# xfause/OpenGL_Ray_Tracing

Hardware: AMD Instinct MI355X
Metric: Mrays/sec + ms/frame (1 spp, 1080p) at 1/2/4/8 MI355X; CPU-ref spp-matched PSNR (higher is better)
Workload: dtype f32; 1 GPU; c2: OpenglRayTracing bunny scene (5k tris), 1080p, 1 spp/frame, Lambert; resolution=1920x1080, spp_per_frame=1, integrator=lambert, max_bounce=2, triangles=5004, bvh_nodes=2826, bvh_builder=sah, env=peppermint, traversal_tree=runtime (checked against uploaded), frame_kernel=path regeneration, frames_in_flight=2, hw_queues=4, frames_per_launch=12, parallelism=screen-tile x1

## Files before the change

opengl_ray_tracing_amd/csrc/pt_kernels.h:

```cpp
#pragma once
#include <hip/hip_runtime.h>
#include <stdint.h>

namespace pt {

#ifndef PT_BLOCK
#define PT_BLOCK 256
#endif
constexpr int BLOCK = PT_BLOCK;
#ifndef PT_LDS_STACK
#define PT_LDS_STACK 32
#endif
#ifndef PT_MIN_WAVES_LAMBERT
#define PT_MIN_WAVES_LAMBERT 3
#endif
#ifndef PT_COST_EMA
#define PT_COST_EMA 2
#endif
#ifndef PT_WIDE_SCENE_MB
#define PT_WIDE_SCENE_MB 48
#endif
constexpr int WIDE_WAVES = 3;
#ifndef PT_WIDE_REGEN_WAVES
#define PT_WIDE_REGEN_WAVES 4
// ... 5 lines not shown
constexpr int wideRegenWaves(int integrator) { return integrator == 2 ? PT_WIDE_REGEN_WAVES : PT_WIDE_REGEN_WAVES_U; }
#ifndef PT_WIDE_REGEN_WAVES_SMALL
#define PT_WIDE_REGEN_WAVES_SMALL 3
#endif
#ifndef PT_MIN_WAVES
#define PT_MIN_WAVES 1
#endif
#ifndef PT_MIN_WAVES_MIS
#define PT_MIN_WAVES_MIS 3
#endif
constexpr int LDS_STACK = PT_LDS_STACK;
#ifndef PT_LDS_NODES
#define PT_LDS_NODES 128
#endif
constexpr int LDS_NODES = PT_LDS_NODES;
#ifndef PT_SPLIT_PCT
#define PT_SPLIT_PCT 25
#endif
#ifndef PT_SPLIT_AUTO
#define PT_SPLIT_AUTO 1
#endif
#ifndef PT_WAVE_TRACE
#define PT_WAVE_TRACE 0
#endif
#ifndef PT_PHASE_STATS
#define PT_PHASE_STATS 0
#endif
constexpr int PHASE_WORDS = 24;
constexpr int WAVE_TRACE_WORDS = PT_PHASE_STATS ? PHASE_WORDS : 6;
#ifndef PT_NUM_QUEUES
#define PT_NUM_QUEUES 32
#endif
constexpr int CTL_LINE_INTS = 64;
constexpr int NUM_QUEUES = PT_NUM_QUEUES;
static_assert((NUM_QUEUES & (NUM_QUEUES - 1)) == 0 && NUM_QUEUES <= 64, "NUM_QUEUES: power of two <= 64");
constexpr int RAY_SHARDS = 64;
constexpr int RAY_SHARD_STRIDE = CTL_LINE_INTS / 2;
constexpr int MAX_SLOTS = 16;
constexpr size_t CTL_QUEUES = 0;
constexpr size_t CTL_STATS = (size_t)MAX_SLOTS * 64 * 256;
constexpr size_t CTL_RAYS = CTL_STATS + 256;
constexpr size_t CTL_BYTES = CTL_RAYS + (size_t)RAY_SHARDS * 256;
#ifndef PT_FAST_TREE
#define PT_FAST_TREE 1
#endif
#ifndef PT_WIDE4
#define PT_WIDE4 2
#endif
#ifndef PT_FUSED_SLABS
#define PT_FUSED_SLABS 1
#endif
#ifndef PT_ACCEL_LEAF
#define PT_ACCEL_LEAF 4
#endif
#ifndef PT_PACKETS
#define PT_PACKETS 1
#endif
constexpr int PKT_DEPTH = 128;
constexpr int PAIR_F4 = 7;
constexpr int HIT_F4 = 4;
constexpr int MAT_F4 = 5;
constexpr int W4_F4 = 8;
constexpr int LEAF_CNT_BITS = 5;
constexpr int REF_NONE = (int)0x80000000;
constexpr int MAX_LEAF = 1 << LEAF_CNT_BITS;
constexpr int MAX_TRIS = (1 << (31 - LEAF_CNT_BITS)) - 1;
// ... 30 lines not shown
  const float2* trig;
  const uint2* light;
  int w, h, res;
  int nt;
};

constexpr int COL_F = 3;
struct FrameRef {
  float* col;
  uint32_t sampleIndex;
};

struct RenderParams {
  SceneView scene;
  Env env;
  int width, height;
  uint32_t frameCounter;
  uint32_t sampleIndex;
  int maxBounce;
  float eye[3];
  float cam[16];
  float4* accum;
  float* col;
  int nFrames;
  uint32_t sampleStride;
  size_t colStride;
  const int* binStart;
  const int* binTris;
  const float4* binGeo;
  const float4* binBox;
  int binTilesX, binTilesY;
  int2* primHit;
  unsigned long long* primMask;
  int zeroQueue;
  int* queue;
  int perQueue;
  int numItems;
  int shardSize;
  int shardTiles;
  int shardsX;
  int rank, world;
  int* ovf;
  int ovfDepth;
  int packets;
  unsigned long long* stats;
  unsigned long long* rayShards;
  const int* tileOrder;
  int orderCap;
  int* tileCost;
  int* tileCostMax;
  unsigned long long* waveTrace;
};

struct TraceParams {
  SceneView scene;
  const float* rays;
  int n;
  float* t;
  int* tri;
  int* ovf;
  int ovfDepth;
};

constexpr int BASIC_MAX_DEPTH = 31;
struct BasicParams {
  const double* shapes;
// ... 53 lines not shown
struct BuildNode {
  float4 lo;
  float4 hi;
  float4 clo;
  float4 chi;
};
struct AccelBuild {
  float4* bvh = nullptr;
  float4* pairs = nullptr;
  int* order = nullptr;
  BuildNode* nodes = nullptr;
  int rootRef = REF_NONE, nDev = 0, depth = 0, nNodes = 0;
};
hipError_t buildAccelDevice(const float4* geo, int nTri, int leafSize, float inflate, float inflateRelAbs,
                            AccelBuild& out, hipStream_t s);
void freeAccelBuild(AccelBuild& a);
hipError_t collapseWide4Device(const BuildNode* nodes, int nNodes, int leafSize, float inflate, float inflateRelAbs,
                               float4** out, int* rootRef, int* nDev, int* depth, hipStream_t s);

hipError_t launchHdrCache(const float* hdr, int w, int h, float4* cache, float* scratch, hipStream_t s);
hipError_t launchEnvCompact(const float4* hdr, const float2* cache, int w, int h, uint2* hdr8, uint32_t* cache4,
                            int* bad, hipStream_t s);
hipError_t launchEnvPack(float4* hdr, const float4* cache, float2* samp, int n, hipStream_t s);
hipError_t launchEnvTrig(float2* trig, int w, int h, hipStream_t s);
hipError_t launchEnvLight(const Env& e, uint2* light, hipStream_t s);
hipError_t launchRender(const RenderParams& p, int integrator, int grid, hipStream_t s, bool cull, bool count,
                        bool wide = false);
constexpr int REORDER_MAX = 4096;
hipError_t launchReorder(int* cost, int* costMax, int* splitLg, int* ema, int* order, int perQueue, int orderCap,
                         int numItems, int group, int numWaves, int splitPct, hipStream_t s);
hipError_t renderBlocksPerCU(int integrator, bool cull, bool count, bool wide, int* nb);
constexpr int PRIM_MISS = -1, PRIM_RETRACE = -2, PRIM_TILE = -3;
hipError_t launchPrimary(const RenderParams& p, hipStream_t s);
struct RegenShape {
  bool wide = false;
  bool fullTree = false;
  bool small = false;
  int block = BLOCK;
  int blocksPerCU = 0;
  size_t dynLds = 0;
};
hipError_t regenShape(int integrator, bool cull, bool wide, int f4nDev, bool smallScene, RegenShape* out);
hipError_t launchRegen(const RenderParams& p, int integrator, int grid, hipStream_t s, bool cull, const RegenShape& r);
int regenLdsStack();
int regenTop4(const RegenShape& r, int integrator);
hipError_t launchTrace(const TraceParams& p, int grid, hipStream_t s, bool cull);
struct GuideParams {
  SceneView scene;
  int width, height;
  float eye[3];
  float cam[16];
  float4* posT;
  float4* nrmTri;
  float4* albedo;
  int* ovf;
  int ovfDepth;
};
hipError_t launchGuides(const GuideParams& p, int grid, hipStream_t s, bool cull);
struct AtrousParams {
  int width, height;
  int stride;
  const float4* in;
  const float4* tmIn;
  const float4* posT;
  const float4* nrmTri;
  const float4* albedo;
  float4* out;
  float4* tmOut;
  float sigmaZ;
  float colDen, albDen;
  int colOn, albOn;
  int normalLog2;
  float limit;
};
constexpr int ATROUS_TILE = 16;
constexpr int ATROUS_LDS_STRIDE = 2;
// ... 70 lines not shown
```

opengl_ray_tracing_amd/csrc/pt_kernels.hip:

```cpp
#include <hip/hip_runtime.h>

#include <stdint.h>

#include "pt_device.h"
#include "pt_kernels.h"
#include "pt_scene.h"
#include "pt_trace.h"

namespace pt {



template <class T>
__device__ V3 pathLambert(T& tr, const Env& env, Hit hit, int maxBounce, uint32_t& seed, Counters& C, bool count) {
  V3 Lo = v3(0, 0, 0), history = v3(1, 1, 1);
  for (int bounce = 0; bounce < maxBounce; bounce++) {
    V3 wi = toNormalHemisphere(sampleHemisphereRand(seed), hit.N);
    Hit nh;
    bool isHit = tr.closest(hit.P, wi, nh);
    float pdf = 1.0f / (2.0f * PT_PI);
    float cosine_i = fmaxf(0.0f, dot(wi, hit.N));
    V3 f_r = hit.m.baseColor / PT_PI;
    if (!isHit) {
      V3 sky = sampleHdr(env, wi);
// ... 243 lines not shown
  __shared__ float4 s_tri[PT_PASS_BIN_CAP * 4];
  __shared__ float4 s_box[PT_PASS_BIN_CAP * 2];
  __shared__ int s_idx[PT_PASS_BIN_CAP];
  const int fr = (int)(blockIdx.x % (unsigned)p.nFrames);
  const int w = (int)(blockIdx.x / (unsigned)p.nFrames);
  const int lane = threadIdx.x;
  if (p.zeroQueue && blockIdx.x == 0)
    for (int q = lane; q < NUM_QUEUES; q += 64) p.queue[q * CTL_LINE_INTS] = 0;
  const int sub = p.shardSize >> 3;
  const int j = w / p.shardTiles, s = w - j * p.shardTiles;
  const int g = j * p.world + p.rank;
  const int gy = g / p.shardsX, gx = g - gy * p.shardsX;
  const int px = gx * p.shardSize + (s % sub) * 8 + (lane & 7);
  const int py = gy * p.shardSize + (s / sub) * 8 + (lane >> 3);
  const bool valid = px < p.width && py < p.height;
  const int tx = (gx * p.shardSize + (s % sub) * 8) >> 3, ty = (gy * p.shardSize + (s / sub) * 8) >> 3;
  int b0 = 0, b1 = 0;
  if (tx < p.binTilesX && ty < p.binTilesY) {
    b0 = p.binStart[ty * p.binTilesX + tx];
    b1 = p.binStart[ty * p.binTilesX + tx + 1];
  }
  const int n = b1 - b0;
  int2* out = p.primHit + ((size_t)fr * p.numItems + w) * 64;
  unsigned long long* mask = p.primMask + (size_t)fr * p.numItems + w;
  FrameRef fp;
  fp.col = p.col ? p.col + (size_t)fr * p.colStride * COL_F : nullptr;
  fp.sampleIndex = p.sampleIndex + (uint32_t)fr * p.sampleStride;
  if (n > PT_PASS_BIN_CAP) {
    const unsigned long long m = __ballot(valid);
    if (valid) out[__popcll(m & ((1ull << lane) - 1ull))] = make_int2(PRIM_TILE, 0);
    if (lane == 0) *mask = m;
    return;
  }
  for (int t = lane >> 2; t < n; t += 16) {
    s_tri[4 * t + (lane & 3)] = p.binGeo[4 * (size_t)(b0 + t) + (lane & 3)];
    if ((lane & 3) < 2) s_box[2 * t + (lane & 3)] = p.binBox[2 * (size_t)(b0 + t) + (lane & 3)];
    else if ((lane & 3) == 2) s_idx[t] = p.binTris[b0 + t];
  }
  __syncthreads();
  uint32_t seed;
  const V3 dir = cameraRay(p, fp.sampleIndex, valid ? px : 0, valid ? py : 0, seed);
  const V3 eye = v3(p.eye[0], p.eye[1], p.eye[2]);
  float tbest = PT_INF;
  int best = -1;
  bool tie = false;
  for (int k = 0; k < n; k++) {
    float tt;
    const bool h = valid && triTest(s_tri[4 * k], s_tri[4 * k + 1], s_tri[4 * k + 2], s_tri[4 * k + 3], eye, dir,
                                    PT_INF, tt);
    if (h && tt == tbest) tie = true;
    if (h && tt < tbest) {
      tbest = tt;
      best = k;
    }
  }
  uint32_t rays = 0;
  int res = PRIM_MISS;
  if (valid) {
    res = best >= 0 ? s_idx[best] : PRIM_MISS;
    if (tie || (res >= 0 && !refReachableBox(p.scene, s_box[2 * best], s_box[2 * best + 1], eye, dir, tbest))) {
      res = PRIM_RETRACE;
    } else {
      rays = 1;
      if (res == PRIM_MISS) {
        Counters C = {0, 0, 0, 0, 0};
        accumulate(p, fp, px, py, sampleHdr(p.env, dir), C, false);
      }
    }
  }
  const bool need = valid && res != PRIM_MISS;
  const unsigned long long m = __ballot(need);
  if (need) out[__popcll(m & ((1ull << lane) - 1ull))] = make_int2(res, __float_as_int(tbest));
  if (lane == 0) *mask = m;
  addRays(p.rayShards, rays);
}

hipError_t launchPrimary(const RenderParams& p, hipStream_t s) {
  if (!p.primHit || !p.primMask || !p.binStart || !p.binGeo || !p.binBox || p.numItems <= 0) return hipErrorInvalidValue;
  hipLaunchKernelGGL(primaryKernel, dim3((unsigned)p.numItems * (unsigned)p.nFrames), dim3(64), 0, s, p);
  return hipGetLastError();
}

template <int INTEG, bool CULL, bool COUNT>
__device__ __forceinline__ void finishPixel(const RenderParams& p, const FrameRef& f, int px, int py, int tri, float t,
                                            Stack& st, Counters& C, const float4* top) {
  Tracer<CULL, COUNT> tr{p.scene, st, C, top};
  uint32_t seed;
  const uint32_t sampleIndex = f.sampleIndex;
  const V3 dir = cameraRay(p, sampleIndex, px, py, seed);
  const V3 eye = v3(p.eye[0], p.eye[1], p.eye[2]);
  Hit first;
  finishHit(p.scene, tri, eye, dir, t, first);
  V3 Li;
  if (INTEG == 0) Li = pathLambert(tr, p.env, first, p.maxBounce, seed, C, COUNT);
  else if (INTEG == 1) Li = pathDisneyUniform(tr, p.env, first, p.maxBounce, seed, C, COUNT);
  else Li = pathMIS(tr, p.env, first, p.maxBounce, seed, px, py, sampleIndex, C, COUNT);
  const V3 Le0 = INTEG == 2 ? emissiveOf(p.scene, tri) : first.m.emissive;
  accumulate(p, f, px, py, Le0 + Li, C, COUNT);
}

struct BHit {
  double distance;
  V3 P, N, color;
  bool emissive;
  double specularRate, roughness, refractRate, refractAngle, refractRoughness;
};
struct BRng {
  uint32_t seed;
  const double* rep;
  long long pos, end;
  bool over;
};
// ... 733 lines not shown
```

opengl_ray_tracing_amd/csrc/pt_regen.hip:

```cpp
#include <hip/hip_runtime.h>
#include <stdint.h>

#include "pt_device.h"
#include "pt_kernels.h"
#include "pt_trace.h"

namespace pt {

#ifndef PT_REGEN_LDS_STACK
#define PT_REGEN_LDS_STACK 16
#endif
constexpr int REGEN_LDS_STACK = PT_REGEN_LDS_STACK;
#ifndef PT_REGEN_YIELD
#define PT_REGEN_YIELD 40
#endif
#ifndef PT_REGEN_MIN_WAVES_U
#define PT_REGEN_MIN_WAVES_U 4
#endif
#ifndef PT_REGEN_MIN_WAVES_MIS
#define PT_REGEN_MIN_WAVES_MIS 1
#endif

#ifndef PT_REGEN_TOP4
#define PT_REGEN_TOP4 128
#endif
#ifndef PT_REGEN_TOP4_3
#define PT_REGEN_TOP4_3 128
#endif
constexpr int regenTop4W(int waves) { return waves == 3 ? PT_REGEN_TOP4_3 : PT_REGEN_TOP4; }

#ifndef PT_TILE_PRIM
#define PT_TILE_PRIM 1
#endif

enum : int { K_NONE = 0, K_PRIMARY = 1, K_BOUNCE = 2, K_SHADOW = 3 };

struct PathState {
  int px, py;
  int fr;
  int kind;
  int bounce;
  uint32_t seed;
  V3 o, d;
  V3 Lo, hist;
  V3 Le0;
  int mat0;
  V3 f_r;
  float cosL;
  float pdfB;
  V3 Lb;
  V3 shC;
  bool haveB;
};

__device__ __forceinline__ uint32_t sampleOf(const RenderParams& p, const PathState& s) {
  return p.sampleIndex + (uint32_t)s.fr * p.sampleStride;
}

__device__ __forceinline__ void writeAccum(const RenderParams& p, const PathState& s, V3 color) {
  const int px = s.px, py = s.py;
  if (p.col) {
    stCol(p.col + ((size_t)s.fr * p.colStride + shareIndex(p, px, py)) * COL_F, color.x, color.y, color.z);
    return;
  }
  float4* a = p.accum + (size_t)py * p.width + px;
  float4 old = ldStream(a);
  float w = 1.0f / (float)(p.frameCounter + 1u);
// ... 135 lines not shown
      float mis_weight = misWeight(s.pdfB, pdf_light);
      V3 cc = ((s.hist * mis_weight) * c) * s.f_r;
      s.Lo = s.Lo + (cc * s.cosL) / s.pdfB;
    } else {
      const float pdf = 1.0f / (2.0f * PT_PI);
      V3 sky = sampleHdr(p.env, s.d);
      s.Lo = s.Lo + ((s.hist * sky) * s.f_r * s.cosL) / pdf;
    }
    color = camEmission<INTEG>(p, s) + s.Lo;
    return false;
  }
  Hit hit;
  finishHit(S, tri, s.o, s.d, t, hit);
  const V3 Le = hit.m.emissive;
  if (primary) {
    if (INTEG == 2) s.mat0 = hit.matId;
    else s.Le0 = Le;
  } else {
    const float pdf = INTEG == 2 ? s.pdfB : 1.0f / (2.0f * PT_PI);
    s.Lo = s.Lo + ((s.hist * Le) * s.f_r * s.cosL) / pdf;
    s.hist = s.hist * ((s.f_r * s.cosL) / pdf);
  }
  if (continueFromHit<INTEG>(p, s, hit, primary ? 0 : s.bounce + 1)) return true;
  color = camEmission<INTEG>(p, s) + s.Lo;
  return false;
}

template <int INTEG, bool CULL, int WAVES = 0, bool W4 = false, int BS = BLOCK, bool FULL = false>
__global__ __launch_bounds__(BS, WAVES > 0 ? WAVES : (INTEG == 2 ? PT_REGEN_MIN_WAVES_MIS : PT_REGEN_MIN_WAVES_U)) void regenKernel(
    RenderParams p) {
  static_assert(!FULL || W4, "the LDS tree is the 4-wide one");
  static_assert(!FULL || PT_REGEN_YIELD > 0, "the whole LDS tree is walked by walk4Run (loadNode4Lds) only");
  constexpr bool TILE_PRIM = PT_TILE_PRIM && INTEG != 2;
  __shared__ int s_stack[REGEN_LDS_STACK * BS];
  StackT<REGEN_LDS_STACK, BS> st;
  st.init(s_stack, p.ovf, p.ovfDepth);
  st.reset();
  __shared__ unsigned s_drained;
  if (threadIdx.x == 0) s_drained = 0;
#if PT_LDS_NODES > 0
  constexpr int TOP4 = regenTop4W(WAVES);
  constexpr int TOPF4 = FULL ? 1 : (W4 && TOP4 * W4_F4 > LDS_NODES * 4) ? TOP4 * W4_F4 : LDS_NODES * 4;
  __shared__ float4 s_nodes[TOPF4];
  extern __shared__ float4 s_tree[];
  if (FULL) {
    const float4* src = p.scene.fbvh4;
    const int n = p.scene.f4nTop * W4_LDS_F4;
    for (int i = threadIdx.x; i < n; i += BS) s_tree[i] = src[W4_F4 * (i / W4_LDS_F4) + i % W4_LDS_F4];
  } else {
    const bool w4 = W4 && p.scene.fast;
    const float4* src = w4 ? p.scene.fbvh4 : p.scene.bvh;
    const int n = w4 ? p.scene.f4nTop * W4_F4 : p.scene.nTop * 4;
    for (int i = threadIdx.x; i < n; i += BS) s_nodes[i] = src[i];
  }
  __syncthreads();
  const float4* top = FULL ? s_tree : s_nodes;
#else
  __syncthreads();
  const float4* top = nullptr;
#endif
  Counters C = {0, 0, 0, 0, 0};
  const int lane = threadIdx.x & 63;
  const int home = blockIdx.x & (NUM_QUEUES - 1);
  const int sub = p.shardSize >> 3;
  TileCursor cur;
  cur.drained = &s_drained;
// ... 25 lines not shown
  const long long phStart = clock64();
#define PH_ADD(k, x)                                                         \
  do {                                                                       \
    const unsigned long long v_ = (unsigned long long)(x);  \
    const unsigned long long m_ = __ballot(1);                               \
    if (__lane_id() == __ffsll((unsigned long long)m_) - 1) ph[k] += v_;     \
  } while (0)
#else
  unsigned long long* ph = nullptr;
#define PH_ADD(k, x) \
  do {               \
  } while (0)
#endif
  while (true) {
#if PT_PHASE_STATS
    const long long phA = clock64();
#endif
    if constexpr (TILE_PRIM) {
      while (true) {
        bool pend = false;
        int2 hP = make_int2(0, 0);
#if PT_PHASE_STATS
        const long long phH = clock64();
#endif
        while (true) {
          PH_ADD(11, 1);
          const unsigned long long idle = __ballot(!active);
          if (idle == 0) break;
          if (cursor >= nValid) {
#if PT_PHASE_STATS
            const long long phC = clock64();
            PH_ADD(17, 1);
#endif
            const int item = cur.next(p.queue, p.perQueue, p.numItems, home, tileFr, p.nFrames);
            if (item < 0) {
              drained = true;
              break;
            }
            tile = item;
#if PT_WAVE_TRACE
            wTiles++;
            wLastClaim = wall_clock64();
#endif
            if (p.primHit) {
              const unsigned long long m = primTileMask(p, tileFr, tile);
              const uint32_t lo = __builtin_amdgcn_readfirstlane((uint32_t)m);
              const uint32_t hi = __builtin_amdgcn_readfirstlane((uint32_t)(m >> 32));
              if ((lane < 32 ? lo >> lane : hi >> (lane - 32)) & 1u)
                s_slot[__builtin_amdgcn_mbcnt_hi(hi, __builtin_amdgcn_mbcnt_lo(lo, 0u))] = (unsigned char)lane;
              nValid = __popc(lo) + __popc(hi);
              if (lane < nValid) s_hit[lane] = primTileEntries(p, tileFr, tile)[lane];
            } else {
              const int px = tilePx(p, tile, sub) + (lane & 7), py = tilePy(p, tile, sub) + (lane >> 3);
              const bool in = px < p.width && py < p.height;
              const unsigned long long valid = __ballot(in);
              if (in) {
                const int k = rankBelow(valid);
                s_slot[k] = (unsigned char)lane;
                s_hit[k] = make_int2(PRIM_RETRACE, 0);
              }
              nValid = __popcll(valid);
            }
            __builtin_amdgcn_fence(__ATOMIC_RELEASE, "wavefront");
            __builtin_amdgcn_wave_barrier();
            __builtin_amdgcn_fence(__ATOMIC_ACQUIRE, "wavefront");
            cursor = 0;
#if PT_PHASE_STATS
            PH_ADD(18, clock64() - phC);
#endif
            continue;
          }
          const int r = cursor + rankBelow(idle);
          if (!active && r < nValid) {
            const int slot = s_slot[r];
            const int2 h = s_hit[r];
            s.px = tilePx(p, tile, sub) + (slot & 7);
            s.py = tilePy(p, tile, sub) + (slot >> 3);
            s.fr = tileFr;
            active = true;
            pend = true;
// ... 2 lines not shown
          cursor = min(nValid, cursor + __popcll(idle));
        }
#if PT_PHASE_STATS
        PH_ADD(16, clock64() - phH);
        const long long phS = clock64();
        if (__ballot(pend)) {
          PH_ADD(21, 1);
          PH_ADD(20, __popcll(__ballot(pend)));
        }
#endif
        bool ended = false;
        if (pend) {
          startPath(p, s);
          if (hP.x >= 0) {
            V3 color;
            if (!advance<INTEG>(p, s, hP.x, __int_as_float(hP.y), color)) {
              writeAccum(p, s, color);
              active = false;
              ended = true;
            }
          }
        }
#if PT_PHASE_STATS
        PH_ADD(19, clock64() - phS);
#endif
        if (drained || __ballot(ended) == 0) break;
      }
    } else {
      while (true) {
        PH_ADD(11, 1);
        const unsigned long long idle = __ballot(!active);
        if (idle == 0) break;
        if (cursor >= 64) {
          const int item = cur.next(p.queue, p.perQueue, p.numItems, home, tileFr, p.nFrames);
          if (item < 0) break;
          tile = item;
          cursor = 0;
          if (p.primHit) {
            const unsigned long long m = primTileMask(p, tileFr, tile);
            tmaskLo = __builtin_amdgcn_readfirstlane((uint32_t)m);
            tmaskHi = __builtin_amdgcn_readfirstlane((uint32_t)(m >> 32));
          }
#if PT_WAVE_TRACE
          wTiles++;
          wLastClaim = wall_clock64();
#endif
        }
        const int slot = cursor + rankBelow(idle);
        if (!active && slot < 64) {
          const int px = tilePx(p, tile, sub) + (slot & 7);
          const int py = tilePy(p, tile, sub) + (slot >> 3);
          int2 h = make_int2(0, 0);
          if (p.primHit)
            h = primOfSlot((unsigned long long)tmaskHi << 32 | tmaskLo, primTileEntries(p, tileFr, tile), slot);
          if (px < p.width && py < p.height && !(p.primHit && h.x == PRIM_MISS)) {
            s.px = px;
            s.py = py;
            s.fr = tileFr;
            startPath(p, s);
            active = true;
            if (p.primHit && h.x >= 0) {
              V3 color;
              if (!advance<INTEG>(p, s, h.x, __int_as_float(h.y), color)) {
                writeAccum(p, s, color);
                active = false;
              }
            }
          }
        }
        cursor = min(64, cursor + __popcll(idle));
      }
    }
#if PT_PHASE_STATS
    PH_ADD(0, clock64() - phA);
#endif
// ... 138 lines not shown
}

template <int I>
static hipError_t launchRegenI(const RenderParams& p, int grid, hipStream_t s, bool cull, const RegenShape& r) {
  if constexpr (I != 2 && PT_REGEN_YIELD > 0) {
    if (r.fullTree) {
      hipLaunchKernelGGL((regenKernel<I, true, wideRegenWaves(I), true, FULL_BS, true>), dim3(grid), dim3(FULL_BS),
                         r.dynLds, s, p);
      return hipGetLastError();
    }
  }
  if (r.fullTree) return hipErrorInvalidValue;
  if constexpr (I == 2 && PT_WIDE_REGEN_WAVES_SMALL != PT_WIDE_REGEN_WAVES)
    if (r.wide && r.small) {
      hipLaunchKernelGGL((regenKernel<I, true, PT_WIDE_REGEN_WAVES_SMALL, true>), dim3(grid), dim3(BLOCK), 0, s, p);
      return hipGetLastError();
    }
  if (r.wide)
    hipLaunchKernelGGL((regenKernel<I, true, wideRegenWaves(I), true>), dim3(grid), dim3(BLOCK), 0, s, p);
  else if (cull) hipLaunchKernelGGL((regenKernel<I, true>), dim3(grid), dim3(BLOCK), 0, s, p);
  else hipLaunchKernelGGL((regenKernel<I, false>), dim3(grid), dim3(BLOCK), 0, s, p);
  return hipGetLastError();
}

hipError_t launchRegen(const RenderParams& p, int integrator, int grid, hipStream_t s, bool cull, const RegenShape& r) {
  if (r.fullTree && p.scene.f4nTop * W4_LDS_F4 * sizeof(float4) > r.dynLds) return hipErrorInvalidValue;
  switch (integrator) {
    case 0: return launchRegenI<0>(p, grid, s, cull, r);
    case 1: return launchRegenI<1>(p, grid, s, cull, r);
    default: return launchRegenI<2>(p, grid, s, cull, r);
  }
}

int regenLdsStack() { return REGEN_LDS_STACK; }
int regenTop4(const RegenShape& r, int integrator) {
  return regenTop4W(r.small ? PT_WIDE_REGEN_WAVES_SMALL : wideRegenWaves(integrator));
}

}
```

opengl_ray_tracing_amd/csrc/pt_runtime.cpp:

```cpp
#include <hip/hip_runtime.h>

#include <algorithm>
#include <array>
#include <map>
#include <chrono>
#include <cmath>
#include <cstdio>
#include <cstdlib>
#include <cstring>
#include <string>
#include <vector>

#include "pt_abi.h"
#include "pt_accel.h"
#include "pt_fmath.h"
#include "pt_kernels.h"
#include "pt_rccl.h"
#include "pt_scene.h"

using namespace pt;

static constexpr int EV_RING = 64;
#ifndef PT_PIPE
#define PT_PIPE 8
// ... 60 lines not shown
  uint32_t* d_cache4 = nullptr;
  uint32_t* d_cacheRow = nullptr;
  unsigned short* d_cacheY = nullptr;
  float2* d_trig = nullptr;
  uint2* d_light = nullptr;
  int hdrW = 0, hdrH = 0;
  double* d_shapes = nullptr;
  int nShapes = 0;
  double* d_basicImg = nullptr;
  double* d_stream = nullptr;
  long long* d_offsets = nullptr;
  long long streamN = 0, nOffsets = 0;
  unsigned long long* d_overruns = nullptr;
  float4* d_accum = nullptr;
  unsigned char* d_ctl = nullptr;
  int* d_ovf = nullptr;
  int* d_cost = nullptr;
  int* d_order = nullptr;
  bool lastFast = false;
  bool lastRegen = false;
  int lastWaves = 0;
  int probeFrame = 0;
  PrimaryBins bins;
  bool binsValid = false;
  float binEye[3] = {}, binCam[16] = {};
  unsigned sceneVersion = 0, binVersion = 0;
  bool pipe = false;
  int pipeDepth = PT_PIPE;
  int pipeDepthBase = PT_PIPE;
  bool pipeDepthFixed = false;
  int batchCap = 1;
  int colCap[COLS] = {};
  int primCap[PIPE] = {};
  int regenWide = -1;
  bool solo = true;
  hipStream_t slotStream[PIPE] = {};
  hipEvent_t kernelDone[PIPE] = {};
  bool slotBusy[PIPE] = {};
  hipEvent_t mixDone[COLS] = {};
  hipStream_t lastMixStream = nullptr;
  hipEvent_t binsBuilt = nullptr;
  unsigned binGen = 0, binGenSeen[MAX_SLOTS] = {};
  float* d_col[COLS] = {};
  int2* d_prim[PIPE] = {};
  int lastSlot = -1;
  int lastCol = -1;
  bool mixPending = false;
  unsigned long long frameNo = 0;
  int probeN[4] = {0, 0, 0, 0};
  double probeMs[4] = {0.0, 0.0, 0.0, 0.0};
  long long probeLast[4] = {-1, -1, -1, -1};
  int probeGen = 0;
  int treeDecided = -1, splitDecided = -1;
  unsigned policyKey = 0, probedKey = ~0u;
  int orderCap = 0;
  bool orderValid[PIPE] = {};
  bool orderSplit[PIPE] = {};
  size_t ovfInts = 0;
  int shardSize = 32, shardsX = 0, shardsY = 0, numItems = 0, perQueue = 0;
  float* d_rays = nullptr;
  float* d_t = nullptr;
  int* d_tri = nullptr;
  size_t traceCap = 0;
  float* d_rgb = nullptr;
  float4* d_guide[3] = {};
  float4* d_guidePN[2][2] = {};
  int guideSet = 0;
  float guideEye[3] = {}, guideCam[16] = {};
  bool guidesValid = false;
  unsigned guideVersion = 0;
  int* d_guideOvf = nullptr;
  size_t guideOvfInts = 0;
  float4* d_dn[2] = {};
  float4* d_dnTm[2] = {};
  const float4* denoised = nullptr;
  float4* d_res[2] = {};
  int resCur = 0;
// ... 243 lines not shown
    ctx->peers.push_back(p);
  }
  if ((rc = createGroup(ctx)) != PT_OK) {
    g_create_err = ctx->err;
    pt_destroy(ctx);
    *out = nullptr;
    return rc;
  }
  return PT_OK;
}

void pt_destroy(pt_ctx* ctx) {
  if (!ctx) return;
  destroyGroup(ctx);
  (void)hipSetDevice(ctx->cfg.device_id);
  if (ctx->own) (void)hipStreamSynchronize(ctx->own);
  dfree(ctx->d_geo); dfree(ctx->d_hit); dfree(ctx->d_mats); dfree(ctx->d_bvh); dfree(ctx->d_pairs);
  dfree(ctx->d_fbvh); dfree(ctx->d_fbvh4); dfree(ctx->d_fpairs); dfree(ctx->d_fastTri);
  dfree(ctx->d_refParent); dfree(ctx->d_refBox); dfree(ctx->d_leafBox);
  dfree(ctx->d_hdr); dfree(ctx->d_cache); dfree(ctx->d_hdr8); dfree(ctx->d_cache4); dfree(ctx->d_shapes);
  dfree(ctx->d_cacheRow); dfree(ctx->d_cacheY); dfree(ctx->d_trig); dfree(ctx->d_light);
  dfree(ctx->d_basicImg); dfree(ctx->d_stream); dfree(ctx->d_offsets); dfree(ctx->d_overruns);
  dfree(ctx->d_accum); dfree(ctx->d_ctl); dfree(ctx->d_ovf); dfree(ctx->d_cost); dfree(ctx->d_order);
  dfree(ctx->d_rays); dfree(ctx->d_t); dfree(ctx->d_tri); dfree(ctx->d_rgb);
  dfree(ctx->d_guide[2]);
  for (auto& set : ctx->d_guidePN) for (auto& g : set) dfree(g);
  dfree(ctx->d_res[0]); dfree(ctx->d_res[1]);
  dfree(ctx->d_mom); dfree(ctx->d_lum); dfree(ctx->d_var0); dfree(ctx->d_lv[0]); dfree(ctx->d_lv[1]);
  dfree(ctx->d_guideOvf); dfree(ctx->d_dn[0]); dfree(ctx->d_dn[1]); dfree(ctx->d_dnTm[0]); dfree(ctx->d_dnTm[1]);
  freePrimaryBins(ctx->bins);
  for (int k = 0; k < PIPE; k++) {
    if (ctx->slotStream[k]) (void)hipStreamSynchronize(ctx->slotStream[k]);
    dfree(ctx->d_prim[k]);
    if (ctx->kernelDone[k]) (void)hipEventDestroy(ctx->kernelDone[k]);
    if (ctx->slotStream[k]) (void)hipStreamDestroy(ctx->slotStream[k]);
  }
  for (int k = 0; k < COLS; k++) {
    dfree(ctx->d_col[k]);
    if (ctx->mixDone[k]) (void)hipEventDestroy(ctx->mixDone[k]);
  }
  if (ctx->binsBuilt) (void)hipEventDestroy(ctx->binsBuilt);
  for (hipEvent_t e : ctx->ev)
    if (e) (void)hipEventDestroy(e);
  if (ctx->own) (void)hipStreamDestroy(ctx->own);
  delete ctx;
}

static inline void nrm3(const float* a, const float* b, const float* c, float N[3]) {
  float e1x = b[0] - a[0], e1y = b[1] - a[1], e1z = b[2] - a[2];
  float e2x = c[0] - a[0], e2y = c[1] - a[1], e2z = c[2] - a[2];
  float cx = e1y * e2z - e2y * e1z;
  float cy = e1z * e2x - e2z * e1x;
  float cz = e1x * e2y - e2x * e1y;
  float inv = 1.0f / std::sqrt((cx * cx + cy * cy) + cz * cz);
  N[0] = cx * inv; N[1] = cy * inv; N[2] = cz * inv;
}

struct WideTree {
  std::vector<float4> bvh;
  int rootRef = REF_NONE, nDev = 0, depth = 0;
};

static std::string encodeWideTree(const float* nodes, int nNodes, int nTri, float inflate, WideTree& out,
                                  float inflateAbs = 0.0f) {
  auto nodeN = [&](int k) { return (int)nodes[(size_t)k * 12 + 3]; };
  auto isInternal = [&](int k) { return k > 0 && k < nNodes && nodeN(k) <= 0; };
// ... 1141 lines not shown
        ctx->binGenSeen[slot] = ctx->binGen;
      }
    }
    if (piped && ctx->binGenSeen[slot] != ctx->binGen) {
      CK(hipStreamWaitEvent(S, ctx->binsBuilt, 0));
      ctx->binGenSeen[slot] = ctx->binGen;
    }
    p.binStart = ctx->bins.binStart;
    p.binTris = ctx->bins.binTris;
    p.binGeo = ctx->bins.binGeo;
    p.binBox = ctx->bins.binBox;
    p.binTilesX = ctx->bins.tilesX;
    p.binTilesY = ctx->bins.tilesY;
    if (pass) {
      const size_t primBytes = shareN * sizeof(int2) + (size_t)ctx->numItems * sizeof(unsigned long long);
      if (piped)
        for (int k = 0; k < D; k++)
          if (!ctx->d_prim[k]) {
            const int cap = std::max(nF, ctx->batchCap);
            CK(hipMalloc(&ctx->d_prim[k], (size_t)cap * primBytes));
            ctx->primCap[k] = cap;
          }
      if (ctx->primCap[slot] < nF) {
        if (ctx->d_prim[slot]) {
          CK(hipStreamSynchronize(S));
          dfree(ctx->d_prim[slot]);
        }
        const int cap = std::max(nF, piped ? ctx->batchCap : 1);
        CK(hipMalloc(&ctx->d_prim[slot], (size_t)cap * primBytes));
        ctx->primCap[slot] = cap;
      }
      p.primHit = ctx->d_prim[slot];
      p.primMask = reinterpret_cast<unsigned long long*>(ctx->d_prim[slot] + (size_t)ctx->primCap[slot] * shareN);
    }
  }
  const bool splitThis = nF == 1;
  p.tileOrder = ordered && ctx->orderValid[slot] && !(!splitThis && ctx->orderSplit[slot]) ? order : nullptr;
  p.orderCap = orderCap;
  p.tileCost = ordered ? cost : nullptr;
  p.tileCostMax = ordered ? cost + ctx->numItems : nullptr;
  if (piped && probing) {
    if (int e = waitOthers()) return e;
  }
  int erc = launchEvents(ctx, &evb, &eve);
  if (erc) return erc;
#if PT_WAVE_TRACE
  const size_t nTrace = (size_t)grid * (bs / 64) * WAVE_TRACE_WORDS;
  unsigned long long* dTrace = nullptr;
  {
    CK(hipMalloc(&dTrace, nTrace * sizeof(unsigned long long)));
    CK(hipMemsetAsync(dTrace, 0, nTrace * sizeof(unsigned long long), S));
  }
  p.waveTrace = dTrace;
#endif
  p.zeroQueue = p.primHit != nullptr;
  if (!p.primHit) CK(hipMemsetAsync(queue, 0, (size_t)NUM_QUEUES * CTL_LINE_INTS * sizeof(int), S));
  CK(hipEventRecord(evb, S));
  if (p.primHit) CK(launchPrimary(p, S));
  if (regen) CK(launchRegen(p, c.integrator, grid, S, cull, rs));
  else CK(launchRender(p, c.integrator, grid, S, cull, count, wide));
#if PT_WAVE_TRACE
  if (dTrace) {
    std::vector<unsigned long long> tr(nTrace);
    CK(hipMemcpyAsync(tr.data(), dTrace, nTrace * sizeof(unsigned long long), hipMemcpyDeviceToHost, S));
    CK(hipStreamSynchronize(S));
    (void)hipFree(dTrace);
    if (const char* fn = std::getenv("PT_WAVE_TRACE_FILE")) {
      if (FILE* f = std::fopen(fn, "ab")) {
        std::fwrite(tr.data(), sizeof(unsigned long long), nTrace, f);
        std::fclose(f);
      }
    }
  }
#endif
  if (ordered) {
    CK(launchReorder(cost, cost + ctx->numItems, cost + 2 * (size_t)ctx->numItems, cost + 3 * (size_t)ctx->numItems,
                     order, ctx->perQueue, orderCap, ctx->numItems, group, grid * (BLOCK / 64), splitThis ? splitPct : 0, S));
    ctx->orderValid[slot] = true;
    ctx->orderSplit[slot] = splitThis && splitPct > 0;
  }
  CK(hipEventRecord(eve, S));
  if (piped) {
    CK(hipEventRecord(ctx->kernelDone[slot], S));
    ctx->slotBusy[slot] = true;
    if (S != ctx->slotStream[slot])
      CK(hipStreamWaitEvent(ctx->slotStream[slot], ctx->kernelDone[slot], 0));
    if (S != ctx->stream) CK(hipStreamWaitEvent(ctx->stream, ctx->kernelDone[slot], 0));
    if (ctx->mixPending && ctx->lastMixStream != ctx->stream)
      CK(hipStreamWaitEvent(ctx->stream, ctx->mixDone[ctx->lastCol], 0));
    ctx->lastMixStream = ctx->stream;
    if (ctx->d_mom) {
// ... 1012 lines not shown
```

opengl_ray_tracing_amd/csrc/pt_trace.h:

```cpp
#pragma once
#include "pt_device.h"
#include "pt_kernels.h"

namespace pt {

struct Counters {
  uint32_t rays, nodes, tris, mats, texels;
};

#ifndef PT_LEAF_WAIT_MK
#define PT_LEAF_WAIT_MK 0
#endif

template <int DEPTH, int STRIDE>
struct StackT {
  static_assert((DEPTH & (DEPTH - 1)) == 0, "LDS stack depth must be a power of two");
  static constexpr int HALF = DEPTH / 2;
  int* lds;
  int* ovf;
  int ovfDepth;
  int sp;
  int base;
  __device__ __forceinline__ void init(int* ldsBase, int* ovfArea, int depth) {
    lds = ldsBase + threadIdx.x;
// ... 666 lines not shown
struct TileCursor {
  int qi = 0;
  unsigned* drained = nullptr;
  __device__ __forceinline__ int next(int* queue, int perQueue, int numItems, int home, int& frame, int nFrames = 1,
                                      const int* order = nullptr, int orderCap = 0) {
    while (qi < NUM_QUEUES) {
      const int q = (home + qi) & (NUM_QUEUES - 1);
      if (drained && qi > 0 &&
          ((__builtin_amdgcn_readfirstlane(*(volatile unsigned*)drained) >> q) & 1u)) {
        qi++;
        continue;
      }
      int it = 0;
      if ((threadIdx.x & 63) == 0) it = atomicAdd(queue + q * CTL_LINE_INTS, 1);
      it = __builtin_amdgcn_readfirstlane(it);
      const int k = nFrames == 1 ? it : it / nFrames;
      if (order) {
        if (it < order[NUM_QUEUES * orderCap + q] * nFrames) {
          frame = it - k * nFrames;
          return order[q * orderCap + k];
        }
      } else {
        const int t = q * perQueue + k;
        if (k < perQueue && t < numItems) {
          frame = it - k * nFrames;
          return t;
        }
      }
      if (drained && (threadIdx.x & 63) == 0) atomicOr(drained, 1u << q);
      qi++;
    }
    return -1;
  }
};

__device__ __forceinline__ size_t shareIndex(const RenderParams& p, int px, int py) {
  const int ss = p.shardSize;
  const int gx = px / ss, gy = py / ss;
  const int j = (gy * p.shardsX + gx) / p.world;
  return (size_t)j * ss * ss + (size_t)((py - gy * ss) * ss + (px - gx * ss));
}

__device__ __forceinline__ unsigned long long primTileMask(const RenderParams& p, int fr, int w) {
  return p.primMask[(size_t)fr * p.numItems + w];
}
__device__ __forceinline__ const int2* primTileEntries(const RenderParams& p, int fr, int w) {
  return p.primHit + ((size_t)fr * p.numItems + w) * 64;
}
__device__ __forceinline__ int2 primOfSlot(unsigned long long m, const int2* e, int slot) {
  if (!((m >> slot) & 1ull)) return make_int2(PRIM_MISS, 0);
  return e[__popcll(m & ((1ull << slot) - 1ull))];
}

__device__ __forceinline__ void addRays(unsigned long long* shards, uint32_t r) {
  for (int off = 32; off > 0; off >>= 1) r += __shfl_down(r, off, 64);
  if ((threadIdx.x & 63) == 0 && r)
    atomicAdd(shards + (blockIdx.x & (RAY_SHARDS - 1)) * RAY_SHARD_STRIDE, (unsigned long long)r);
}

struct Hit {
  V3 P, N, viewDir;
  Material m;
  int matId;
};
__device__ __forceinline__ V3 emissiveMat(const SceneView& S, int matId) {
  const float4* m = S.mats + MAT_F4 * (size_t)matId;
// ... 102 lines not shown
```

Baseline: 20200 Mrays/s.

## Compact non-empty tiles into per-queue live lists before regen kernel

Adds a liveListKernel that scans primary-hit masks per queue and writes a compacted list of (tile, frame, mask) entries for tiles that have at least one live pixel. The regen kernel's work hand-out then claims entries from this list via nextLive, which skips empty (all-miss) tiles and reads the mask through the scalar constant path instead of a separate load. It also skips the bin load and barrier in the primary kernel when a bin is empty. The cost is one extra small kernel launch per batch, extra device buffers, and host-side allocation logic.

```diff
diff --git a/opengl_ray_tracing_amd/csrc/pt_kernels.h b/opengl_ray_tracing_amd/csrc/pt_kernels.h
--- a/opengl_ray_tracing_amd/csrc/pt_kernels.h
+++ b/opengl_ray_tracing_amd/csrc/pt_kernels.h
@@ -61,6 +61,8 @@
 #define PT_NUM_QUEUES 32
 #endif
 constexpr int CTL_LINE_INTS = 64;
+constexpr int LIVE_HEAD = 16;
+__host__ __device__ constexpr int liveStride(int perQueue, int nFrames) { return LIVE_HEAD + ((perQueue * nFrames + 15) & ~15); }
 constexpr int NUM_QUEUES = PT_NUM_QUEUES;
 static_assert((NUM_QUEUES & (NUM_QUEUES - 1)) == 0 && NUM_QUEUES <= 64, "NUM_QUEUES: power of two <= 64");
 constexpr int RAY_SHARDS = 64;
@@ -157,6 +159,7 @@
   int binTilesX, binTilesY;
   int2* primHit;
   unsigned long long* primMask;
+  uint4* liveItems;
   int zeroQueue;
   int* queue;
   int perQueue;
@@ -276,6 +279,7 @@
 hipError_t renderBlocksPerCU(int integrator, bool cull, bool count, bool wide, int* nb);
 constexpr int PRIM_MISS = -1, PRIM_RETRACE = -2, PRIM_TILE = -3;
 hipError_t launchPrimary(const RenderParams& p, hipStream_t s);
+hipError_t launchLiveList(const RenderParams& p, hipStream_t s);
 struct RegenShape {
   bool wide = false;
   bool fullTree = false;
@@ -286,6 +290,7 @@
 };
 hipError_t regenShape(int integrator, bool cull, bool wide, int f4nDev, bool smallScene, RegenShape* out);
 hipError_t launchRegen(const RenderParams& p, int integrator, int grid, hipStream_t s, bool cull, const RegenShape& r);
+bool regenTakesLists(int integrator, const RegenShape& r);
 int regenLdsStack();
 int regenTop4(const RegenShape& r, int integrator);
 hipError_t launchTrace(const TraceParams& p, int grid, hipStream_t s, bool cull);
diff --git a/opengl_ray_tracing_amd/csrc/pt_kernels.hip b/opengl_ray_tracing_amd/csrc/pt_kernels.hip
--- a/opengl_ray_tracing_amd/csrc/pt_kernels.hip
+++ b/opengl_ray_tracing_amd/csrc/pt_kernels.hip
@@ -299,12 +299,14 @@
     if (lane == 0) *mask = m;
     return;
   }
-  for (int t = lane >> 2; t < n; t += 16) {
-    s_tri[4 * t + (lane & 3)] = p.binGeo[4 * (size_t)(b0 + t) + (lane & 3)];
-    if ((lane & 3) < 2) s_box[2 * t + (lane & 3)] = p.binBox[2 * (size_t)(b0 + t) + (lane & 3)];
-    else if ((lane & 3) == 2) s_idx[t] = p.binTris[b0 + t];
-  }
-  __syncthreads();
+  if (n > 0) {
+    for (int t = lane >> 2; t < n; t += 16) {
+      s_tri[4 * t + (lane & 3)] = p.binGeo[4 * (size_t)(b0 + t) + (lane & 3)];
+      if ((lane & 3) < 2) s_box[2 * t + (lane & 3)] = p.binBox[2 * (size_t)(b0 + t) + (lane & 3)];
+      else if ((lane & 3) == 2) s_idx[t] = p.binTris[b0 + t];
+    }
+    __syncthreads();
+  }
   uint32_t seed;
   const V3 dir = cameraRay(p, fp.sampleIndex, valid ? px : 0, valid ? py : 0, seed);
   const V3 eye = v3(p.eye[0], p.eye[1], p.eye[2]);
@@ -345,6 +347,51 @@
 hipError_t launchPrimary(const RenderParams& p, hipStream_t s) {
   if (!p.primHit || !p.primMask || !p.binStart || !p.binGeo || !p.binBox || p.numItems <= 0) return hipErrorInvalidValue;
   hipLaunchKernelGGL(primaryKernel, dim3((unsigned)p.numItems * (unsigned)p.nFrames), dim3(64), 0, s, p);
+  return hipGetLastError();
+}
+
+constexpr int LIVE_BS = 1024;
+__global__ __launch_bounds__(LIVE_BS) void liveListKernel(RenderParams p) {
+  __shared__ int s_wave[LIVE_BS / 64];
+  const int q = blockIdx.x, lane = threadIdx.x & 63, wv = threadIdx.x >> 6;
+  const int nF = p.nFrames, total = p.perQueue * nF;
+  uint4* seg = p.liveItems + (size_t)q * liveStride(p.perQueue, nF);
+  uint4* out = seg + LIVE_HEAD;
+  auto load = [&](int it, int& t, int& fr) -> unsigned long long {
+    const int k = it / nF;
+    fr = it - k * nF;
+    t = q * p.perQueue + k;
+    return it < total && t < p.numItems ? p.primMask[(size_t)fr * p.numItems + t] : 0ull;
+  };
+  int base = 0;
+  int t, fr;
+  unsigned long long m = load((int)threadIdx.x, t, fr);
+  for (int it0 = 0; it0 < total; it0 += LIVE_BS) {
+    int tn, frn;
+    const unsigned long long mn = load(it0 + LIVE_BS + (int)threadIdx.x, tn, frn);
+    const unsigned long long b = __ballot(m != 0);
+    if (lane == 0) s_wave[wv] = __popcll(b);
+    __syncthreads();
+    int before = 0, all = 0;
+    for (int w = 0; w < LIVE_BS / 64; w++) {
+      const int c = s_wave[w];
+      before += w < wv ? c : 0;
+      all += c;
+    }
+    if (m != 0)
+      out[base + before + __popcll(b & ((1ull << lane) - 1ull))] = make_uint4((uint32_t)t, (uint32_t)fr, (uint32_t)m, (uint32_t)(m >> 32));
+    base += all;
+    __syncthreads();
+    m = mn;
+    t = tn;
+    fr = frn;
+  }
+  if (threadIdx.x == 0) seg[0] = make_uint4((uint32_t)base, 0u, 0u, 0u);
+}
+
+hipError_t launchLiveList(const RenderParams& p, hipStream_t s) {
+  if (!p.primMask || !p.liveItems || p.numItems <= 0) return hipErrorInvalidValue;
+  hipLaunchKernelGGL(liveListKernel, dim3(NUM_QUEUES), dim3(LIVE_BS), 0, s, p);
   return hipGetLastError();
 }
 
diff --git a/opengl_ray_tracing_amd/csrc/pt_regen.hip b/opengl_ray_tracing_amd/csrc/pt_regen.hip
--- a/opengl_ray_tracing_amd/csrc/pt_regen.hip
+++ b/opengl_ray_tracing_amd/csrc/pt_regen.hip
@@ -33,6 +33,9 @@
 #define PT_TILE_PRIM 1
 #endif
 
+constexpr bool regenLists(int integ, int waves) {
+  return !(integ == 2 && waves == PT_WIDE_REGEN_WAVES && PT_WIDE_REGEN_WAVES_SMALL != PT_WIDE_REGEN_WAVES);
+}
 enum : int { K_NONE = 0, K_PRIMARY = 1, K_BOUNCE = 2, K_SHADOW = 3 };
 
 struct PathState {
@@ -234,6 +237,7 @@
   static_assert(!FULL || W4, "the LDS tree is the 4-wide one");
   static_assert(!FULL || PT_REGEN_YIELD > 0, "the whole LDS tree is walked by walk4Run (loadNode4Lds) only");
   constexpr bool TILE_PRIM = PT_TILE_PRIM && INTEG != 2;
+  constexpr bool LISTS = regenLists(INTEG, WAVES);
   __shared__ int s_stack[REGEN_LDS_STACK * BS];
   StackT<REGEN_LDS_STACK, BS> st;
   st.init(s_stack, p.ovf, p.ovfDepth);
@@ -325,20 +329,18 @@
             const long long phC = clock64();
             PH_ADD(17, 1);
 #endif
-            const int item = cur.next(p.queue, p.perQueue, p.numItems, home, tileFr, p.nFrames);
-            if (item < 0) {
+            uint32_t lo = 0, hi = 0;
+            static_assert(LISTS, "the tile hand-out's variants all take live lists");
+            if (!cur.nextLive(p.queue, p.primHit ? p.liveItems : nullptr, p.perQueue, p.numItems, p.nFrames, home, tile,
+                              tileFr, lo, hi)) {
               drained = true;
               break;
             }
-            tile = item;
 #if PT_WAVE_TRACE
             wTiles++;
             wLastClaim = wall_clock64();
 #endif
             if (p.primHit) {
-              const unsigned long long m = primTileMask(p, tileFr, tile);
-              const uint32_t lo = __builtin_amdgcn_readfirstlane((uint32_t)m);
-              const uint32_t hi = __builtin_amdgcn_readfirstlane((uint32_t)(m >> 32));
               if ((lane < 32 ? lo >> lane : hi >> (lane - 32)) & 1u)
                 s_slot[__builtin_amdgcn_mbcnt_hi(hi, __builtin_amdgcn_mbcnt_lo(lo, 0u))] = (unsigned char)lane;
               nValid = __popc(lo) + __popc(hi);
@@ -407,15 +409,21 @@
         const unsigned long long idle = __ballot(!active);
         if (idle == 0) break;
         if (cursor >= 64) {
-          const int item = cur.next(p.queue, p.perQueue, p.numItems, home, tileFr, p.nFrames);
-          if (item < 0) break;
-          tile = item;
+          if constexpr (LISTS) {
+            if (!cur.nextLive(p.queue, p.primHit ? p.liveItems : nullptr, p.perQueue, p.numItems, p.nFrames, home, tile,
+                              tileFr, tmaskLo, tmaskHi))
+              break;
+          } else {
+            const int item = cur.next(p.queue, p.perQueue, p.numItems, home, tileFr, p.nFrames);
+            if (item < 0) break;
+            tile = item;
+            if (p.primHit) {
+              const unsigned long long m = primTileMask(p, tileFr, tile);
+              tmaskLo = __builtin_amdgcn_readfirstlane((uint32_t)m);
+              tmaskHi = __builtin_amdgcn_readfirstlane((uint32_t)(m >> 32));
+            }
+          }
           cursor = 0;
-          if (p.primHit) {
-            const unsigned long long m = primTileMask(p, tileFr, tile);
-            tmaskLo = __builtin_amdgcn_readfirstlane((uint32_t)m);
-            tmaskHi = __builtin_amdgcn_readfirstlane((uint32_t)(m >> 32));
-          }
 #if PT_WAVE_TRACE
           wTiles++;
           wLastClaim = wall_clock64();
@@ -620,6 +628,9 @@
   }
 }
 
+bool regenTakesLists(int integrator, const RegenShape& r) {
+  return regenLists(integrator, r.wide ? (r.small ? PT_WIDE_REGEN_WAVES_SMALL : wideRegenWaves(integrator)) : 0);
+}
 int regenLdsStack() { return REGEN_LDS_STACK; }
 int regenTop4(const RegenShape& r, int integrator) {
   return regenTop4W(r.small ? PT_WIDE_REGEN_WAVES_SMALL : wideRegenWaves(integrator));
diff --git a/opengl_ray_tracing_amd/csrc/pt_runtime.cpp b/opengl_ray_tracing_amd/csrc/pt_runtime.cpp
--- a/opengl_ray_tracing_amd/csrc/pt_runtime.cpp
+++ b/opengl_ray_tracing_amd/csrc/pt_runtime.cpp
@@ -116,6 +116,7 @@
   int batchCap = 1;
   int colCap[COLS] = {};
   int primCap[PIPE] = {};
+  int liveCap[PIPE] = {};
   int regenWide = -1;
   bool solo = true;
   hipStream_t slotStream[PIPE] = {};
@@ -127,6 +128,7 @@
   unsigned binGen = 0, binGenSeen[MAX_SLOTS] = {};
   float* d_col[COLS] = {};
   int2* d_prim[PIPE] = {};
+  uint4* d_live[PIPE] = {};
   int lastSlot = -1;
   int lastCol = -1;
   bool mixPending = false;
@@ -436,6 +438,7 @@
   for (int k = 0; k < PIPE; k++) {
     if (ctx->slotStream[k]) (void)hipStreamSynchronize(ctx->slotStream[k]);
     dfree(ctx->d_prim[k]);
+    dfree(ctx->d_live[k]);
     if (ctx->kernelDone[k]) (void)hipEventDestroy(ctx->kernelDone[k]);
     if (ctx->slotStream[k]) (void)hipStreamDestroy(ctx->slotStream[k]);
   }
@@ -1643,6 +1646,26 @@
       }
       p.primHit = ctx->d_prim[slot];
       p.primMask = reinterpret_cast<unsigned long long*>(ctx->d_prim[slot] + (size_t)ctx->primCap[slot] * shareN);
+      if (regen && regenTakesLists(c.integrator, rs)) {
+        auto liveBytes = [&](int cap) { return (size_t)NUM_QUEUES * liveStride(ctx->perQueue, cap) * sizeof(uint4); };
+        if (piped)
+          for (int k = 0; k < D; k++)
+            if (!ctx->d_live[k]) {
+              const int cap = std::max(nF, ctx->batchCap);
+              CK(hipMalloc(&ctx->d_live[k], liveBytes(cap)));
+              ctx->liveCap[k] = cap;
+            }
+        if (ctx->liveCap[slot] < nF) {
+          if (ctx->d_live[slot]) {
+            CK(hipStreamSynchronize(S));
+            dfree(ctx->d_live[slot]);
+          }
+          const int cap = std::max(nF, piped ? ctx->batchCap : 1);
+          CK(hipMalloc(&ctx->d_live[slot], liveBytes(cap)));
+          ctx->liveCap[slot] = cap;
+        }
+        p.liveItems = p.primHit ? ctx->d_live[slot] : nullptr;
+      }
     }
   }
   const bool splitThis = nF == 1;
@@ -1668,6 +1691,7 @@
   if (!p.primHit) CK(hipMemsetAsync(queue, 0, (size_t)NUM_QUEUES * CTL_LINE_INTS * sizeof(int), S));
   CK(hipEventRecord(evb, S));
   if (p.primHit) CK(launchPrimary(p, S));
+  if (p.liveItems) CK(launchLiveList(p, S));
   if (regen) CK(launchRegen(p, c.integrator, grid, S, cull, rs));
   else CK(launchRender(p, c.integrator, grid, S, cull, count, wide));
 #if PT_WAVE_TRACE
diff --git a/opengl_ray_tracing_amd/csrc/pt_trace.h b/opengl_ray_tracing_amd/csrc/pt_trace.h
--- a/opengl_ray_tracing_amd/csrc/pt_trace.h
+++ b/opengl_ray_tracing_amd/csrc/pt_trace.h
@@ -722,6 +722,40 @@
     }
     return -1;
   }
+  __device__ __forceinline__ bool nextLive(int* queue, const uint4* live, int perQueue, int numItems, int nFrames,
+                                           int home, int& tile, int& frame, uint32_t& maskLo, uint32_t& maskHi) {
+    typedef const __attribute__((address_space(4))) uint32_t* ConstU32;
+    while (qi < NUM_QUEUES) {
+      const int q = (home + qi) & (NUM_QUEUES - 1);
+      const bool gone = drained && qi > 0 && ((__builtin_amdgcn_readfirstlane(*(volatile unsigned*)drained) >> q) & 1u);
+      if (!gone) {
+        const uint4* seg = live + (size_t)q * liveStride(perQueue, nFrames);
+        int n = 0;
+        if (live) n = (int)*(ConstU32)seg;
+        int it = 0;
+        if ((threadIdx.x & 63) == 0) it = atomicAdd(queue + q * CTL_LINE_INTS, 1);
+        it = __builtin_amdgcn_readfirstlane(it);
+        n = live ? __builtin_amdgcn_readfirstlane(n) : min(perQueue, numItems - q * perQueue) * nFrames;
+        if (it < n) {
+          if (live) {
+            ConstU32 r = (ConstU32)(seg + LIVE_HEAD + it);
+            tile = (int)r[0];
+            frame = (int)r[1];
+            maskLo = r[2];
+            maskHi = r[3];
+          } else {
+            const int k = it / nFrames;
+            tile = q * perQueue + k;
+            frame = it - k * nFrames;
+          }
+          return true;
+        }
+        if (drained && (threadIdx.x & 63) == 0) atomicOr(drained, 1u << q);
+      }
+      qi++;
+    }
+    return false;
+  }
 };
 
 __device__ __forceinline__ size_t shareIndex(const RenderParams& p, int px, int py) {
```

Measured after the change: 21180 Mrays/s, median of 6. +4.8%, better.
